# haidog-yaqub/EzAudio

Measured on AMD Instinct MI355X. Metric: denoising steps/sec (EzAudio-XL, 10 s latent, CFG on), higher is better.
Workload: dtype bf16

## Files before the change

ezaudio_amd/csrc/attn.hip:

```cpp
#include "common.h"

namespace {

typedef __attribute__((ext_vector_type(4))) short s16x4;

__device__ __forceinline__ float pair_max(float x) {
    const auto r = __builtin_amdgcn_permlane32_swap(__float_as_uint(x), __float_as_uint(x), false, false);
    return fmaxf(__uint_as_float(r[0]), __uint_as_float(r[1]));
}
__device__ __forceinline__ float pair_sum(float x) {
    const auto r = __builtin_amdgcn_permlane32_swap(__float_as_uint(x), __float_as_uint(x), false, false);
    return __uint_as_float(r[0]) + __uint_as_float(r[1]);
}

template <int DH>
struct HeadGeom;
template <>
struct HeadGeom<64> { static constexpr int DQK = 64, DV = 64; };
template <>
struct HeadGeom<72> { static constexpr int DQK = 80, DV = 96; };

template <int DH, int NKH, bool ZQ = false, int QT = 64>
__global__ __launch_bounds__(128 * NKH) void k_attn(AttnArgs a) {
    static_assert(QT == 64 || (QT == 32 && NKH == 4), "32-query tiles: the 8-wave fused-projection form only");
    constexpr int NQS = QT / 32;
    constexpr int NT = 128 * NKH;
    constexpr int TK = 32 * NKH;
    constexpr int DQK = HeadGeom<DH>::DQK;
    constexpr int DV = HeadGeom<DH>::DV;
    constexpr int NKS = DQK / 16;
    constexpr int NDT = DV / 32;
    constexpr int KSTR = DQK * 2 + 16;
    constexpr int VSTR = 192;
    static_assert(DV * 2 <= VSTR, "V row");
    constexpr int KBYTES = TK * KSTR, VBYTES = TK * VSTR;
    constexpr int BUF = KBYTES + VBYTES;
    constexpr int KCH = TK * DQK * 2 / 16;
    constexpr int VCPR = DV / 8;
    constexpr int VCH = TK * VCPR;
    constexpr int KPT = (KCH + NT - 1) / NT, VPT = (VCH + NT - 1) / NT;
    static_assert(KPT <= 3 && VPT <= 3, "staging registers");
    constexpr int DN = DV >= 96 ? 96 : 64;
    constexpr int DW = DQK;
    constexpr int DS = DQK;
    constexpr int NRS = QT == 64 ? 3 : 4;
    constexpr int PSTAGE = (QT + DN) * 128, PRING = 2 * NRS * PSTAGE;
    constexpr int PRED = 4 * 64 * DS * 4, PQS = QT * DQK * 2;
    constexpr int SMEM = NKH == 4 ? (2 * BUF > PRED + PQS ? (2 * BUF > PRING ? 2 * BUF : PRING) : (PRED + PQS > PRING ? PRED + PQS : PRING)) : 2 * BUF;
    constexpr int ZX = ZQ ? QT * 8 + 2 * DQK * 4 : 0;
    __shared__ __attribute__((aligned(16))) char smem[SMEM + ZX];

    int Lq_ = a.Lq;
    asm("" : "+s"(Lq_) : "s"(a.q), "s"(a.k), "s"(a.v), "s"(a.kmask), "s"(a.out), "s"(a.ldo), "s"(a.B), "s"(a.H), "s"(a.Lk), "s"(a.Lqp), "s"(a.Lkp), "s"(a.xu), "s"(a.ldu),
        "s"(a.xw), "s"(a.ldw), "s"(a.xw_rows), "s"(a.xK), "s"(a.xcd_map), "s"(a.nq), "s"(a.ppx), "s"(a.mnq), "s"(a.mH), "s"(a.q_raw), "s"(a.ts), "s"(a.xk2), "s"(a.zstat_in),
        "s"(a.zs_stride), "s"(a.zparts));
    const int tid = threadIdx.x;
    const int lane = tid & 63;
    const int wave = tid >> 6;
    const int qs = QT == 64 ? (wave & 1) : 0, kh = QT == 64 ? (wave >> 1) : (wave & 3);
    const bool active = QT == 64 || __builtin_amdgcn_readfirstlane(wave) < 4;
    const int r32 = lane & 31, hi = lane >> 5;
    int qt, h, b;
    if (a.xcd_map) {
        const int xcd = blockIdx.x & 7, sl = blockIdx.x >> 3;
        const int sq = ez_div(sl, a.mnq);
        const int pair = xcd * a.ppx + sq;
        qt = sl - sq * a.nq;
        if (pair >= a.B * a.H) return;
        b = ez_div(pair, a.mH); h = pair - b * a.H;
    } else {
        qt = blockIdx.x; h = blockIdx.y; b = blockIdx.z;
    }
    const int q0 = qt * QT + qs * 32;
    const long bh = (long)b * a.H + h;
    unsigned long long* ts = (a.ts && tid < 64) ? a.ts + 8 * (long)blockIdx.x : nullptr;
    if (ts && lane == 0) { ts[0] = __builtin_readcyclecounter(); ts[6] = ez_stamp_start(); }

    const bf16_t* Q = a.q + (bh * a.Lqp + q0 + r32) * DQK + 8 * hi;
    const char* Kg = reinterpret_cast<const char*>(a.k + bh * a.Lkp * DQK);
    const bf16_t* Vg = a.v + bh * DV * (long)a.Lkp;
    const uint8_t* km = a.kmask ? a.kmask + (long)b * a.Lk : nullptr;

    bf16x8 qf[NKS];
    if (NKH == 4 && a.xu) {
        if constexpr (NKH == 4) {
            constexpr int FN = DN / 32;
            constexpr int NPART = QT == 64 ? 4 : 8;
            const int rowb = b * a.Lq;
            float2* zrow_l = reinterpret_cast<float2*>(smem + SMEM);
            float* zgc_l = reinterpret_cast<float*>(smem + SMEM + QT * 8);
            ZStatRegs zst;
            float4 zgc_reg = make_float4(0.f, 0.f, 0.f, 0.f);
            const int wave_u = __builtin_amdgcn_readfirstlane(wave);
            const char* gA = reinterpret_cast<const char*>(a.xu);
            const char* gW = reinterpret_cast<const char*>(a.xw);
            const int nt = a.xK / 64;
            auto z_request = [&]() {
                if constexpr (ZQ) {
                    if (tid < 4 * QT) {
                        int qr = qt * QT + (tid >> 2);
                        qr = qr < a.Lq ? qr : a.Lq - 1;
                        z_row_stats_load(a.zstat_in + (rowb + qr), a.zs_stride, a.zparts, tid & 3, zst);
                    }
                    if (tid < 2 * (DH / 4)) {
                        const int which = tid >= DH / 4, t4 = tid - which * (DH / 4);
                        zgc_reg = *reinterpret_cast<const float4*>((which ? a.zC : a.zG) + h * DH + 4 * t4);
                    }
                }
            };
            f32x16 acc[FN];
#pragma unroll
            for (int j = 0; j < FN; ++j)
#pragma unroll
                for (int r = 0; r < 16; ++r) acc[j][r] = 0.f;
            if constexpr (QT == 32) {
                constexpr int NCH = (32 + DW) * 8, NW1 = (NCH - NT) / 64;
                static_assert(NCH > NT && NCH <= 2 * NT && (NCH - NT) % 64 == 0, "two passes, whole waves");
                uint32_t off0, off1;
                {
                    const int row = tid >> 3, c = tid & 7;
                    if (row < 32) {
                        int grow = rowb + qt * 32 + row;
                        grow = grow < rowb + a.Lq - 1 ? grow : rowb + a.Lq - 1;
                        off0 = (uint32_t)(grow * a.ldu + ((c ^ ((row >> 1) & 7)) << 3)) * 2u;
                    } else {
                        const int r2 = row - 32;
                        int gr = h * DH + r2;
                        gr = gr < a.xw_rows - 1 ? gr : a.xw_rows - 1;
                        off0 = (uint32_t)(gr * a.ldw + ((c ^ ((r2 >> 1) & 7)) << 3)) * 2u;
                    }
                    const int r2 = (tid >> 3) + 32;
                    int gr = h * DH + r2;
                    gr = gr < a.xw_rows - 1 ? gr : a.xw_rows - 1;
                    off1 = (uint32_t)(gr * a.ldw + ((c ^ ((r2 >> 1) & 7)) << 3)) * 2u;
                }
                const char* g0 = wave_u < 4 ? gA : gW;
                const bool two = wave_u < NW1;
                auto stage2 = [&](int sidx) {
                    char* dst = smem + (sidx % NRS) * 2 * PSTAGE + wave_u * 1024;
#pragma unroll
                    for (int sub = 0; sub < 2; ++sub) {
                        const long ko = (long)(2 * sidx + sub) * 128;
                        __builtin_amdgcn_global_load_lds((const __attribute__((address_space(1))) void*)(g0 + ko + off0),
                                                         (__attribute__((address_space(3))) void*)(dst + sub * PSTAGE), 16, 0, 0);
                        if (two)
                            __builtin_amdgcn_global_load_lds((const __attribute__((address_space(1))) void*)(gW + ko + off1),
                                                             (__attribute__((address_space(3))) void*)(dst + sub * PSTAGE + NT * 16), 16, 0, 0);
                    }
                };
                const int ns = nt >> 1;
                stage2(0);
                z_request();
                if (ns > 1) stage2(1);
                if (ns > 2) stage2(2);
                const int sub = wave_u >> 2, kq = wave_u & 3;
                const uint32_t fo = r32 * 128 + (((2 * kq + hi) ^ ((r32 >> 1) & 7)) << 4);
                for (int sidx = 0; sidx < ns; ++sidx) {
                    const int younger = ns - 1 - sidx < NRS - 2 ? ns - 1 - sidx : NRS - 2;
                    if (two) {
                        if (younger >= 2) asm volatile("s_waitcnt vmcnt(8)" ::: "memory");
                        else if (younger == 1) asm volatile("s_waitcnt vmcnt(4)" ::: "memory");
                        else asm volatile("s_waitcnt vmcnt(0)" ::: "memory");
                    } else {
                        if (younger >= 2) asm volatile("s_waitcnt vmcnt(4)" ::: "memory");
                        else if (younger == 1) asm volatile("s_waitcnt vmcnt(2)" ::: "memory");
                        else asm volatile("s_waitcnt vmcnt(0)" ::: "memory");
                    }
                    __builtin_amdgcn_s_barrier();
                    if (sidx + NRS - 1 < ns) stage2(sidx + NRS - 1);
                    const char* cT = smem + (sidx % NRS) * 2 * PSTAGE + sub * PSTAGE;
                    const bf16x8 af = *reinterpret_cast<const bf16x8*>(cT + fo);
#pragma unroll
                    for (int j = 0; j < FN; ++j) {
                        const bf16x8 bfr = *reinterpret_cast<const bf16x8*>(cT + 32 * 128 + fo + j * 4096);
                        acc[j] = __builtin_amdgcn_mfma_f32_32x32x16_bf16(bfr, af, acc[j], 0, 0, 0);
                    }
#pragma unroll
                    for (int j = 0; j < FN; ++j) asm volatile("" : "+a"(acc[j]));
                }
            } else {
            const int mh = wave & 1, kq = wave >> 1;
            uint32_t aoff[1], boff[(DW * 8 + NT - 1) / NT];
            stage_offsets<64, NT>(aoff, a.ldu, rowb + qt * 64, rowb + a.Lq - 1, tid);
            stage_offsets<DW, NT>(boff, a.ldw, h * DH, a.xw_rows - 1, tid);
            auto stage = [&](int t) {
                char* dst = smem + (t % 3) * PSTAGE + wave_u * 1024;
                stage_tile<64, NT>(gA + (long)t * 128, aoff, dst, tid);
                stage_tile<DW, NT>(gW + (long)t * 128, boff, dst + 64 * 128, tid);
            };
            const bool two = (DW * 8 > NT) && (wave_u * 64 + NT < DW * 8);
            stage(0);
            if (nt > 1) stage(1);
            z_request();
            const uint32_t fo = r32 * 128 + (((2 * kq + hi) ^ ((r32 >> 1) & 7)) << 4);
            if (a.xk2 && (nt & 1) == 0) {
                const int ns = nt >> 1;
                auto stage2 = [&](int sidx) {
                    char* dst = smem + (sidx % 3) * 2 * PSTAGE + wave_u * 1024;
#pragma unroll
                    for (int sub = 0; sub < 2; ++sub) {
                        stage_tile<64, NT>(gA + (long)(2 * sidx + sub) * 128, aoff, dst + sub * PSTAGE, tid);
                        stage_tile<DW, NT>(gW + (long)(2 * sidx + sub) * 128, boff, dst + sub * PSTAGE + 64 * 128, tid);
                    }
                };
                if (ns > 1) stage2(1);
                for (int sidx = 0; sidx < ns; ++sidx) {
                    if (sidx + 1 < ns) {
                        if (two) asm volatile("s_waitcnt vmcnt(6)" ::: "memory"); else asm volatile("s_waitcnt vmcnt(4)" ::: "memory");
                    } else {
                        asm volatile("s_waitcnt vmcnt(0)" ::: "memory");
                    }
                    __builtin_amdgcn_s_barrier();
                    if (sidx + 2 < ns) stage2(sidx + 2);
#pragma unroll
                    for (int sub = 0; sub < 2; ++sub) {
                        const char* cT = smem + (sidx % 3) * 2 * PSTAGE + sub * PSTAGE;
                        const bf16x8 af = *reinterpret_cast<const bf16x8*>(cT + fo + mh * 4096);
#pragma unroll
                        for (int j = 0; j < FN; ++j) {
                            const bf16x8 bfr = *reinterpret_cast<const bf16x8*>(cT + 64 * 128 + fo + j * 4096);
                            acc[j] = __builtin_amdgcn_mfma_f32_32x32x16_bf16(bfr, af, acc[j], 0, 0, 0);
                        }
                    }
#pragma unroll
                    for (int j = 0; j < FN; ++j) asm volatile("" : "+a"(acc[j]));
                }
            } else
            for (int t = 0; t < nt; ++t) {
                if (t + 1 < nt) {
                    if (two) asm volatile("s_waitcnt vmcnt(3)" ::: "memory"); else asm volatile("s_waitcnt vmcnt(2)" ::: "memory");
                } else {
                    asm volatile("s_waitcnt vmcnt(0)" ::: "memory");
                }
                __builtin_amdgcn_s_barrier();
                if (t + 2 < nt) stage(t + 2);
                const char* cT = smem + (t % 3) * PSTAGE;
                const bf16x8 af = *reinterpret_cast<const bf16x8*>(cT + fo + mh * 4096);
#pragma unroll
                for (int j = 0; j < FN; ++j) {
                    const bf16x8 bfr = *reinterpret_cast<const bf16x8*>(cT + 64 * 128 + fo + j * 4096);
                    acc[j] = __builtin_amdgcn_mfma_f32_32x32x16_bf16(bfr, af, acc[j], 0, 0, 0);
                }
#pragma unroll
                for (int j = 0; j < FN; ++j) asm volatile("" : "+a"(acc[j]));
            }
            }
#pragma unroll
            for (int j = 0; j < FN; ++j) asm volatile("s_nop 7\n\ts_nop 7\n\ts_nop 3" : "+a"(acc[j]));
            if constexpr (ZQ) {
                if (tid < 4 * QT) {
                    const float2 mr = z_row_stats_finish(zst, a.zparts, tid & 3, a.zD, a.zeps);
                    if ((tid & 3) == 0) zrow_l[tid >> 2] = mr;
                }
                if (tid < 2 * (DH / 4)) {
                    const int which = tid >= DH / 4, t4 = tid - which * (DH / 4);
                    *reinterpret_cast<float4*>(zgc_l + which * DQK + 4 * t4) = zgc_reg;
                }
            }
            __syncthreads();
            float* red = reinterpret_cast<float*>(smem);
            {
                const int pw = QT == 64 ? (wave >> 1) : wave, prow = QT == 64 ? 32 * (wave & 1) + r32 : r32;
#pragma unroll
                for (int j = 0; j < FN; ++j)
#pragma unroll
                    for (int g = 0; g < 4; ++g) {
                        const int col = 32 * j + 8 * g + 4 * hi;
                        if (col < DS)
                            *reinterpret_cast<float4*>(red + ((pw * QT + prow) * DS + col)) =
                                make_float4(acc[j][4 * g], acc[j][4 * g + 1], acc[j][4 * g + 2], acc[j][4 * g + 3]);
                    }
            }
            __syncthreads();
            if (QT == 64 || tid < 8 * QT) {
                constexpr int CP = DH / 8;
                bf16_t* qs_l = reinterpret_cast<bf16_t*>(smem + PRED);
                const int row = tid >> 3, part = tid & 7;
                float v[CP];
                float s1 = 0.f;
                const float2 zmr = ZQ ? zrow_l[row] : make_float2(0.f, 1.f);
                const float zmu = zmr.x, zr = zmr.y;
#pragma unroll
                for (int e = 0; e < CP; ++e) {
                    const int col = part * CP + e;
                    if constexpr (QT == 64) {
                        v[e] = red[(0 * 64 + row) * DS + col] + red[(1 * 64 + row) * DS + col] + red[(2 * 64 + row) * DS + col] +
                               red[(3 * 64 + row) * DS + col];
                    } else {
                        float t = red[row * DS + col];
#pragma unroll
                        for (int w = 1; w < NPART; ++w) t += red[(w * QT + row) * DS + col];
                        v[e] = t;
                    }
                    if constexpr (ZQ) v[e] = fmaf(zr, v[e], fmaf(-zr * zmu, zgc_l[col], zgc_l[DQK + col]));
                    s1 += v[e];
                }
                s1 = oct_sum(s1);
                const float mean = s1 * (1.f / DH);
                float s2 = 0.f;
#pragma unroll
                for (int e = 0; e < CP; ++e) { const float d = v[e] - mean; s2 += d * d; }
                s2 = oct_sum(s2);
                const float rstd = rsqrtf(s2 * (1.f / DH) + 1e-5f);
#pragma unroll
                for (int e = 0; e < CP; ++e) {
                    const int col = part * CP + e;
                    qs_l[row * DQK + col] = f2bf((v[e] - mean) * rstd * a.qn_w[col] + a.qn_b[col]);
                }
                if (DQK > DH && part == 0)
                    for (int col = DH; col < DQK; ++col) qs_l[row * DQK + col] = 0;
            }
            __syncthreads();
            {
                const bf16_t* qs_l = reinterpret_cast<const bf16_t*>(smem + PRED);
#pragma unroll
                for (int ks = 0; ks < NKS; ++ks) qf[ks] = *reinterpret_cast<const bf16x8*>(qs_l + (32 * qs + r32) * DQK + 16 * ks + 8 * hi);
            }
            __syncthreads();
        }
    } else if (a.q_raw) {
        int qr = q0 + r32;
        if (qr >= a.Lq) qr = a.Lq - 1;
        const float* src = a.q_raw + ((long)b * a.Lq + qr) * a.ld_qraw + h * DH + 8 * hi;
        float v[NKS][8];
        float s = 0.f;
#pragma unroll
        for (int ks = 0; ks < NKS; ++ks) {
            const bool ok = 16 * ks + 8 * hi < DH;
            const float4 lo = ok ? *reinterpret_cast<const float4*>(src + 16 * ks) : make_float4(0.f, 0.f, 0.f, 0.f);
            const float4 hh = ok ? *reinterpret_cast<const float4*>(src + 16 * ks + 4) : make_float4(0.f, 0.f, 0.f, 0.f);
            v[ks][0] = lo.x; v[ks][1] = lo.y; v[ks][2] = lo.z; v[ks][3] = lo.w;
            v[ks][4] = hh.x; v[ks][5] = hh.y; v[ks][6] = hh.z; v[ks][7] = hh.w;
#pragma unroll
            for (int e = 0; e < 8; ++e) s += v[ks][e];
        }
        s += __shfl_xor(s, 32, 64);
        const float mean = s * (1.f / DH);
        float q2 = 0.f;
#pragma unroll
        for (int ks = 0; ks < NKS; ++ks)
            if (16 * ks + 8 * hi < DH) {
#pragma unroll
                for (int e = 0; e < 8; ++e) { const float d = v[ks][e] - mean; q2 += d * d; }
            }
        q2 += __shfl_xor(q2, 32, 64);
        const float rstd = rsqrtf(q2 * (1.f / DH) + 1e-5f);
#pragma unroll
        for (int ks = 0; ks < NKS; ++ks) {
            const int d0 = 16 * ks + 8 * hi;
            const bool ok = d0 < DH;
            const int dw = ok ? d0 : 0;
            union { bf16x8 v; uint32_t u[4]; } pk;
#pragma unroll
            for (int e = 0; e < 4; ++e) {
                const float y0 = ok ? (v[ks][2 * e] - mean) * rstd * a.qn_w[dw + 2 * e] + a.qn_b[dw + 2 * e] : 0.f;
                const float y1 = ok ? (v[ks][2 * e + 1] - mean) * rstd * a.qn_w[dw + 2 * e + 1] + a.qn_b[dw + 2 * e + 1] : 0.f;
                pk.u[e] = pack_bf2(y0, y1);
            }
            qf[ks] = pk.v;
        }
    } else {
#pragma unroll
        for (int ks = 0; ks < NKS; ++ks) qf[ks] = *reinterpret_cast<const bf16x8*>(Q + 16 * ks);
    }

    uint4 k0 = {}, k1 = {}, k2 = {}, v0 = {}, v1 = {}, v2 = {};
    uint32_t koff[3], voff[3];
#pragma unroll
    for (int i = 0; i < 3; ++i) {
        int ck = tid + NT * i, cv = tid + NT * i;
        ck = ck < KCH ? ck : KCH - 1;
        cv = cv < VCH ? cv : VCH - 1;
        koff[i] = (uint32_t)ck * 16u;
        voff[i] = (uint32_t)cv * 16u;
    }
    const __amdgpu_buffer_rsrc_t krs = __builtin_amdgcn_make_buffer_rsrc(const_cast<char*>(Kg), 0, a.Lkp * DQK * 2, 0x00020000);
    const __amdgpu_buffer_rsrc_t vrs = __builtin_amdgcn_make_buffer_rsrc(const_cast<bf16_t*>(Vg), 0, DV * a.Lkp * 2, 0x00020000);
    auto kchunk = [&](int i, int key0) -> uint4 {
        return __builtin_bit_cast(uint4, __builtin_amdgcn_raw_buffer_load_b128(krs, (int)koff[i], key0 * DQK * 2, 0));
    };
    auto vchunk = [&](int i, int key0) -> uint4 {
        return __builtin_bit_cast(uint4, __builtin_amdgcn_raw_buffer_load_b128(vrs, (int)voff[i], key0 * DV * 2, 0));
    };
    auto kstore = [&](int i, char* kb, const uint4& val) {
        const int c = tid + NT * i;
        if (c < KCH) *reinterpret_cast<uint4*>(kb + (c / (DQK / 8)) * KSTR + (c % (DQK / 8)) * 16) = val;
    };
    auto vstore = [&](int i, char* vb, const uint4& val) {
        const int c = tid + NT * i;
        if (c < VCH) *reinterpret_cast<uint4*>(vb + (c / VCPR) * VSTR + (c % VCPR) * 16) = val;
    };
#define LOAD_TILE(t)                                   \
    do {                                               \
        const int key0_ = (t) * TK;                    \
        k0 = kchunk(0, key0_);                         \
        k1 = kchunk(1, key0_);                         \
        if constexpr (KPT > 2) k2 = kchunk(2, key0_);  \
        v0 = vchunk(0, key0_);                         \
        v1 = vchunk(1, key0_);                         \
        if constexpr (VPT > 2) v2 = vchunk(2, key0_);  \
    } while (0)
#define WRITE_TILE(buf)                                \
    do {                                               \
        char* kb_ = smem + (buf) * BUF;                \
        char* vb_ = kb_ + KBYTES;                      \
        kstore(0, kb_, k0);                            \
        kstore(1, kb_, k1);                            \
        if constexpr (KPT > 2) kstore(2, kb_, k2);     \
        vstore(0, vb_, v0);                            \
        vstore(1, vb_, v1);                            \
        if constexpr (VPT > 2) vstore(2, vb_, v2);     \
    } while (0)

    f32x16 o[NDT];
#pragma unroll
    for (int t = 0; t < NDT; ++t)
#pragma unroll
        for (int r = 0; r < 16; ++r) o[t][r] = 0.f;
    float m = -1e30f, lsum = 0.f;
    constexpr float RESCALE_THR = 4.0f;
    const float c = 1.4426950408889634f * rsqrtf((float)DH);

    if (NKH == 4 && __builtin_amdgcn_readfirstlane(threadIdx.x) >= 256) __builtin_amdgcn_s_setprio(1);
    const int ntiles = (a.Lk + TK - 1) / TK;
    LOAD_TILE(0);
    WRITE_TILE(0);
    __syncthreads();
    if (ts && lane == 0) ts[1] = __builtin_readcyclecounter();
    for (int t = 0; t < ntiles; ++t) {
        if (t + 1 < ntiles) LOAD_TILE(t + 1);
        const char* kb = smem + (t & 1) * BUF;
        const char* vb = kb + KBYTES;
        const char* vtr = vb + (32 * kh + 4 * hi + ((lane & 15) >> 2)) * VSTR + ((lane & 16) + 4 * (lane & 3)) * 2;
        const int key0 = t * TK + kh * 32;
        if (active && key0 < a.Lk) {
            const int kidx = key0 + r32;
            bool kv = kidx < a.Lk;
            if (km) kv = kv && (km[kidx < a.Lk ? kidx : 0] != 0);
            const uint32_t ball = (uint32_t)__ballot(kv);
            const uint32_t tmask = ball >> (4 * hi);
            const bool full = ball == 0xffffffffu;
            f32x16 s;
            {
                const bf16x8 kf0 = *reinterpret_cast<const bf16x8*>(kb + (kh * 32 + r32) * KSTR + hi * 16);
                asm("s_nop 1\n\tv_mfma_f32_32x32x16_bf16 %0, %1, %2, 0" : "=&v"(s) : "v"(kf0), "v"(qf[0]));
            }
#pragma unroll
            for (int ks = 1; ks < NKS; ++ks) {
                const bf16x8 kf = *reinterpret_cast<const bf16x8*>(kb + (kh * 32 + r32) * KSTR + (2 * ks + hi) * 16);
                if (ks + 1 < NKS) asm("s_nop 1\n\tv_mfma_f32_32x32x16_bf16 %0, %1, %2, %0" : "+v"(s) : "v"(kf), "v"(qf[ks]));
                else asm("s_nop 1\n\tv_mfma_f32_32x32x16_bf16 %0, %1, %2, %0\n\ts_nop 7\n\ts_nop 7\n\ts_nop 3" : "+v"(s) : "v"(kf), "v"(qf[ks]));
            }
            float tmax = -1e30f;
            if (full) {
#pragma unroll
                for (int r = 0; r < 16; ++r) tmax = fmaxf(tmax, s[r]);
                tmax *= c;
            } else {
#pragma unroll
                for (int r = 0; r < 16; ++r) {
                    const bool v = (tmask >> ((r & 3) + 8 * (r >> 2))) & 1u;
                    s[r] = v ? s[r] * c : -1e30f;
                    tmax = fmaxf(tmax, s[r]);
                }
            }
            tmax = pair_max(tmax);
            if (!__all(tmax <= m + RESCALE_THR)) {
                const float mnew = fmaxf(m, tmax);
                const float alpha = __builtin_amdgcn_exp2f(m - mnew);
                m = mnew;
                lsum *= alpha;
#pragma unroll
                for (int tt = 0; tt < NDT; ++tt)
#pragma unroll
                    for (int r = 0; r < 16; ++r) o[tt][r] *= alpha;
            }
            float psum = 0.f;
            float p[16];
            if (full) {
                const f32x2 c2 = {c, c}, nm2 = {-m, -m};
                f32x2 ps2 = {0.f, 0.f};
#pragma unroll
                for (int r = 0; r < 16; r += 2) {
                    f32x2 x = {s[r], s[r + 1]};
                    x = __builtin_elementwise_fma(x, c2, nm2);
                    p[r] = __builtin_amdgcn_exp2f(x[0]);
                    p[r + 1] = __builtin_amdgcn_exp2f(x[1]);
                    const f32x2 pp = {p[r], p[r + 1]};
                    ps2 += pp;
                }
                psum = ps2[0] + ps2[1];
            } else {
#pragma unroll
                for (int r = 0; r < 16; ++r) {
                    const bool v = (tmask >> ((r & 3) + 8 * (r >> 2))) & 1u;
                    p[r] = v ? __builtin_amdgcn_exp2f(s[r] - m) : 0.f;
                    psum += p[r];
                }
            }
            psum = pair_sum(psum);
            lsum += psum;
#pragma unroll
            for (int step = 0; step < 2; ++step) {
                union { bf16x8 v; uint32_t u[4]; } pf;
#pragma unroll
                for (int e = 0; e < 4; ++e) pf.u[e] = pack_bf2(p[8 * step + 2 * e], p[8 * step + 2 * e + 1]);
#pragma unroll
                for (int tt = 0; tt < NDT; ++tt) {
                    const char* vp = vtr + (16 * step) * VSTR + 64 * tt;
                    union { bf16x8 v; s16x4 h2[2]; } vf;
                    vf.h2[0] = __builtin_amdgcn_ds_read_tr16_b64_v4i16((__attribute__((address_space(3))) s16x4*)(vp));
                    vf.h2[1] = __builtin_amdgcn_ds_read_tr16_b64_v4i16((__attribute__((address_space(3))) s16x4*)(vp + 8 * VSTR));
                    asm("s_nop 1\n\tv_mfma_f32_32x32x16_bf16 %0, %1, %2, %0" : "+v"(o[tt]) : "v"(vf.v), "v"(pf.v));
                }
            }
        }
        if (t + 1 < ntiles) WRITE_TILE((t + 1) & 1);
        __syncthreads();
    }

    if (ts && lane == 0) ts[2] = __builtin_readcyclecounter();
#pragma unroll
    for (int tt = 0; tt < NDT; ++tt) asm volatile("s_nop 7\n\ts_nop 7\n\ts_nop 3" : "+v"(o[tt]));
    constexpr int NG = DH / 8;
    constexpr int NW = 2 * NKH;
    float4* xo = reinterpret_cast<float4*>(smem);
    float* xml = reinterpret_cast<float*>(smem + NKH * NQS * NG * 64 * 16);
    static_assert(SMEM >= NKH * NQS * NG * 64 * 16 + NKH * NQS * 2 * 32 * 4, "exchange area must fit the staging buffers");
    if (active) {
#pragma unroll
        for (int G = 0; G < NG; ++G)
            xo[((kh * NQS + qs) * NG + G) * 64 + lane] = make_float4(o[G / 4][4 * (G % 4)], o[G / 4][4 * (G % 4) + 1], o[G / 4][4 * (G % 4) + 2], o[G / 4][4 * (G % 4) + 3]);
        if (hi == 0) {
            xml[((kh * NQS + qs) * 2 + 0) * 32 + r32] = m;
            xml[((kh * NQS + qs) * 2 + 1) * 32 + r32] = lsum;
        }
    }
    __syncthreads();
    if (ts && lane == 0) ts[4] = __builtin_readcyclecounter();
    float wgt[NKH];
    {
        float mk[NKH], mm = -1e30f;
#pragma unroll
        for (int k = 0; k < NKH; ++k) { mk[k] = xml[((k * NQS + qs) * 2 + 0) * 32 + r32]; mm = fmaxf(mm, mk[k]); }
        float l = 0.f;
#pragma unroll
        for (int k = 0; k < NKH; ++k) { wgt[k] = __builtin_amdgcn_exp2f(mk[k] - mm); l = fmaf(xml[((k * NQS + qs) * 2 + 1) * 32 + r32], wgt[k], l); }
        const float inv = 1.f / l;
#pragma unroll
        for (int k = 0; k < NKH; ++k) wgt[k] *= inv;
    }
    const int qrow = q0 + r32;
    bf16_t* orow = a.out + ((long)b * a.Lq + (qrow < a.Lq ? qrow : a.Lq - 1)) * a.ldo + h * DH + 4 * hi;
#pragma unroll
    for (int i = 0; i < (NQS * NG + NW - 1) / NW; ++i) {
        const int G = (wave + i * NW) / NQS;
        if (G < NG) {
            float4 acc = make_float4(0.f, 0.f, 0.f, 0.f);
#pragma unroll
            for (int k = 0; k < NKH; ++k) {
                const float4 v = xo[((k * NQS + qs) * NG + G) * 64 + lane];
                acc.x = fmaf(v.x, wgt[k], acc.x); acc.y = fmaf(v.y, wgt[k], acc.y); acc.z = fmaf(v.z, wgt[k], acc.z); acc.w = fmaf(v.w, wgt[k], acc.w);
            }
            if (qrow < a.Lq) {
                uint2 v;
                v.x = pack_bf2(acc.x, acc.y);
                v.y = pack_bf2(acc.z, acc.w);
                if (a.wt) st8_wt(orow + 8 * G, v); else *reinterpret_cast<uint2*>(orow + 8 * G) = v;
            }
        }
    }
    if (ts && lane == 0) { asm volatile("s_waitcnt vmcnt(0)" ::: "memory"); ts[3] = __builtin_readcyclecounter(); ts[7] = __builtin_amdgcn_s_memrealtime(); }
}

#undef LOAD_TILE
#undef WRITE_TILE

}

int launch_attention(const AttnArgs& a0, hipStream_t st) {
    AttnArgs a = a0;
    if (a.b0 > 0) {
        const int DQK = a.dh == 64 ? 64 : 80, DV = a.dh == 64 ? 64 : 96;
        const long b0 = a.b0;
        if (a.q) a.q += b0 * a.H * a.Lqp * DQK;
        if (a.k) a.k += b0 * a.H * a.Lkp * DQK;
        if (a.v) a.v += b0 * a.H * DV * (long)a.Lkp;
        if (a.kmask) a.kmask += b0 * a.Lk;
        if (a.out) a.out += b0 * a.Lq * a.ldo;
        if (a.q_raw) a.q_raw += b0 * a.Lq * a.ld_qraw;
        if (a.xu) a.xu += b0 * a.Lq * a.ldu;
        if (a.zstat_in) a.zstat_in += b0 * a.Lq;
        a.b0 = 0;
    }
    const long nwg64 = (long)((a.Lq + 63) / 64) * a.H * a.B;
    int nkh = a.nkh;
    if (nkh != 2 && nkh != 4) nkh = nwg64 <= 512 ? 4 : 2;
    if (a.Lkp % 128) nkh = 2;
    if (a.xu && nkh != 4) return 1;
    if (a.dh != 64 && a.dh != 72) return 1;
    const bool zq = a.xu && a.zstat_in;
    if (zq && !(a.zG && a.zC && a.zparts > 0 && a.zparts <= Z_MAXP && a.zs_stride > 0 && a.zw > 0)) return 1;
    const bool q32 = zq && nkh == 4 && (a.xK / 64) % 2 == 0 && a.xcd_map && (a.qtile == 32 || (a.qtile == 0 && nwg64 <= 128));
    const int QT = q32 ? 32 : 64;
    a.nq = (a.Lq + QT - 1) / QT;
    a.ppx = (a.B * a.H + 7) / 8;
    a.mnq = ez_magic(a.nq); a.mH = ez_magic(a.H);
    dim3 grid(a.nq, a.H, a.B);
    if (a.xcd_map) grid = dim3(8 * a.ppx * a.nq, 1, 1);
    if (a.ts && (long)grid.x * grid.y * grid.z > a.ts_cap) a.ts = nullptr;
    if (q32) {
        if (a.dh == 64) hipLaunchKernelGGL((k_attn<64, 4, true, 32>), grid, dim3(512), 0, st, a);
        else hipLaunchKernelGGL((k_attn<72, 4, true, 32>), grid, dim3(512), 0, st, a);
        return 0;
    }
    if (a.dh == 64) {
        if (nkh == 4 && zq) hipLaunchKernelGGL((k_attn<64, 4, true>), grid, dim3(512), 0, st, a);
        else if (nkh == 4) hipLaunchKernelGGL((k_attn<64, 4>), grid, dim3(512), 0, st, a);
        else hipLaunchKernelGGL((k_attn<64, 2>), grid, dim3(256), 0, st, a);
    } else {
        if (nkh == 4 && zq) hipLaunchKernelGGL((k_attn<72, 4, true>), grid, dim3(512), 0, st, a);
        else if (nkh == 4) hipLaunchKernelGGL((k_attn<72, 4>), grid, dim3(512), 0, st, a);
        else hipLaunchKernelGGL((k_attn<72, 2>), grid, dim3(256), 0, st, a);
    }
    return 0;
}
```

Before: 263.6.

## Restructure fused Q-projection staging into per-wave k-chunks with barrier-free pipelining

For the 32-query fused projection path, each wave now owns whole 64-wide k-chunks in its own LDS slot, with two waves double-buffered. This replaces the shared 3/4-stage ring that needed a block barrier every step. All fragment reads are issued before the next chunk's async global-to-LDS load, and the z-statistics loads are folded into the vmcnt accounting. The cross-wave partial-sum reduction moves to a swizzled float4 layout with vectorized reads and packed bf16 stores, and one syncthreads is dropped. Explicit s_nop padding after the MFMAs adds fixed stall cycles, and the more complex vmcnt bookkeeping risks subtle ordering bugs.

```diff
diff --git a/ezaudio_amd/csrc/attn.hip b/ezaudio_amd/csrc/attn.hip
--- a/ezaudio_amd/csrc/attn.hip
+++ b/ezaudio_amd/csrc/attn.hip
@@ -43,10 +43,17 @@
     constexpr int DN = DV >= 96 ? 96 : 64;
     constexpr int DW = DQK;
     constexpr int DS = DQK;
-    constexpr int NRS = QT == 64 ? 3 : 4;
-    constexpr int PSTAGE = (QT + DN) * 128, PRING = 2 * NRS * PSTAGE;
-    constexpr int PRED = 4 * 64 * DS * 4, PQS = QT * DQK * 2;
-    constexpr int SMEM = NKH == 4 ? (2 * BUF > PRED + PQS ? (2 * BUF > PRING ? 2 * BUF : PRING) : (PRED + PQS > PRING ? PRED + PQS : PRING)) : 2 * BUF;
+    constexpr int PSTAGE = (64 + DN) * 128, PRING = 2 * 3 * PSTAGE;
+    constexpr int NPC = (32 + DW) / 8;
+    constexpr int CHUNK = NPC * 1024, SLOT = (32 + DN) * 128, NX = 2;
+    constexpr int PSLOTS = 8 * SLOT + NX * CHUNK + (DN - DW) * 128;
+    constexpr int RP = 24;
+    constexpr int PPART = QT == 64 ? 64 * RP * 16 : SLOT;
+    constexpr int PRED = QT == 64 ? 4 * PPART : 8 * SLOT, PQS = QT * DQK * 2;
+    static_assert(QT == 64 || 32 * RP * 16 <= SLOT, "a wave's partial tile must fit its slot");
+    static_assert(DS / 4 <= RP && RP % 8 == 0, "partial rows");
+    constexpr int PPROJ = QT == 64 ? (PRED + PQS > PRING ? PRED + PQS : PRING) : (PSLOTS > PRED + PQS ? PSLOTS : PRED + PQS);
+    constexpr int SMEM = NKH == 4 ? (2 * BUF > PPROJ ? 2 * BUF : PPROJ) : 2 * BUF;
     constexpr int ZX = ZQ ? QT * 8 + 2 * DQK * 4 : 0;
     __shared__ __attribute__((aligned(16))) char smem[SMEM + ZX];
 
@@ -108,75 +115,88 @@
                     }
                 }
             };
+            auto z_request_all = [&]() {
+                if constexpr (ZQ) {
+                    int qr = qt * QT + ((tid >> 2) & (QT - 1));
+                    qr = qr < a.Lq ? qr : a.Lq - 1;
+                    z_row_stats_load(a.zstat_in + (rowb + qr), a.zs_stride, a.zparts, tid & 3, zst);
+                    const int tc = tid < 2 * (DH / 4) ? tid : 2 * (DH / 4) - 1;
+                    const int which = tc >= DH / 4, t4 = tc - which * (DH / 4);
+                    zgc_reg = *reinterpret_cast<const float4*>((which ? a.zC : a.zG) + h * DH + 4 * t4);
+                }
+            };
             f32x16 acc[FN];
 #pragma unroll
             for (int j = 0; j < FN; ++j)
 #pragma unroll
                 for (int r = 0; r < 16; ++r) acc[j][r] = 0.f;
             if constexpr (QT == 32) {
-                constexpr int NCH = (32 + DW) * 8, NW1 = (NCH - NT) / 64;
-                static_assert(NCH > NT && NCH <= 2 * NT && (NCH - NT) % 64 == 0, "two passes, whole waves");
-                uint32_t off0, off1;
-                {
-                    const int row = tid >> 3, c = tid & 7;
-                    if (row < 32) {
+                constexpr int NZ = ZQ ? Z_PT + 1 : 0;
+                static_assert(NZ + NPC < 64, "vmcnt is a 6-bit counter");
+                uint32_t poff[NPC];
+#pragma unroll
+                for (int p = 0; p < NPC; ++p) {
+                    const int row = 8 * p + (lane >> 3), c = lane & 7;
+                    if (p < 4) {
                         int grow = rowb + qt * 32 + row;
                         grow = grow < rowb + a.Lq - 1 ? grow : rowb + a.Lq - 1;
-                        off0 = (uint32_t)(grow * a.ldu + ((c ^ ((row >> 1) & 7)) << 3)) * 2u;
+                        poff[p] = (uint32_t)(grow * a.ldu + ((c ^ ((row >> 1) & 7)) << 3)) * 2u;
                     } else {
                         const int r2 = row - 32;
                         int gr = h * DH + r2;
                         gr = gr < a.xw_rows - 1 ? gr : a.xw_rows - 1;
-                        off0 = (uint32_t)(gr * a.ldw + ((c ^ ((r2 >> 1) & 7)) << 3)) * 2u;
-                    }
-                    const int r2 = (tid >> 3) + 32;
-                    int gr = h * DH + r2;
-                    gr = gr < a.xw_rows - 1 ? gr : a.xw_rows - 1;
-                    off1 = (uint32_t)(gr * a.ldw + ((c ^ ((r2 >> 1) & 7)) << 3)) * 2u;
-                }
-                const char* g0 = wave_u < 4 ? gA : gW;
-                const bool two = wave_u < NW1;
-                auto stage2 = [&](int sidx) {
-                    char* dst = smem + (sidx % NRS) * 2 * PSTAGE + wave_u * 1024;
-#pragma unroll
-                    for (int sub = 0; sub < 2; ++sub) {
-                        const long ko = (long)(2 * sidx + sub) * 128;
-                        __builtin_amdgcn_global_load_lds((const __attribute__((address_space(1))) void*)(g0 + ko + off0),
-                                                         (__attribute__((address_space(3))) void*)(dst + sub * PSTAGE), 16, 0, 0);
-                        if (two)
-                            __builtin_amdgcn_global_load_lds((const __attribute__((address_space(1))) void*)(gW + ko + off1),
-                                                             (__attribute__((address_space(3))) void*)(dst + sub * PSTAGE + NT * 16), 16, 0, 0);
-                    }
+                        poff[p] = (uint32_t)(gr * a.ldw + ((c ^ ((r2 >> 1) & 7)) << 3)) * 2u;
+                    }
+                }
+                auto issue = [&](int c, char* dst) {
+                    const long ko = (long)c * 128;
+#pragma unroll
+                    for (int p = 0; p < NPC; ++p)
+                        __builtin_amdgcn_global_load_lds((const __attribute__((address_space(1))) void*)((p < 4 ? gA : gW) + ko + poff[p]),
+                                                         (__attribute__((address_space(3))) void*)(dst + p * 1024), 16, 0, 0);
                 };
-                const int ns = nt >> 1;
-                stage2(0);
-                z_request();
-                if (ns > 1) stage2(1);
-                if (ns > 2) stage2(2);
-                const int sub = wave_u >> 2, kq = wave_u & 3;
-                const uint32_t fo = r32 * 128 + (((2 * kq + hi) ^ ((r32 >> 1) & 7)) << 4);
-                for (int sidx = 0; sidx < ns; ++sidx) {
-                    const int younger = ns - 1 - sidx < NRS - 2 ? ns - 1 - sidx : NRS - 2;
-                    if (two) {
-                        if (younger >= 2) asm volatile("s_waitcnt vmcnt(8)" ::: "memory");
-                        else if (younger == 1) asm volatile("s_waitcnt vmcnt(4)" ::: "memory");
+                const int nmine = wave_u < nt ? (nt - wave_u + 7) >> 3 : 0;
+                const bool two = wave_u < NX;
+                char* const slot0 = smem + wave_u * SLOT;
+                char* const slot1 = smem + 8 * SLOT + (two ? wave_u : 0) * CHUNK;
+                if (nmine > 0) issue(wave_u, slot0);
+                __builtin_amdgcn_sched_barrier(0);
+                z_request_all();
+                __builtin_amdgcn_sched_barrier(0);
+                if (two && nmine > 1) issue(wave_u + 8, slot1);
+                __builtin_amdgcn_sched_barrier(0);
+                uint32_t fo[4];
+#pragma unroll
+                for (int ks = 0; ks < 4; ++ks) fo[ks] = r32 * 128 + (((2 * ks + hi) ^ ((r32 >> 1) & 7)) << 4);
+                for (int i = 0; i < nmine; ++i) {
+                    const bool nxt = two && i + 1 < nmine;
+                    if (i == 0) {
+                        if (nxt) asm volatile("s_waitcnt vmcnt(%0)" ::"n"(NZ + NPC) : "memory");
+                        else asm volatile("s_waitcnt vmcnt(%0)" ::"n"(NZ) : "memory");
+                    } else {
+                        if (nxt) asm volatile("s_waitcnt vmcnt(%0)" ::"n"(NPC) : "memory");
                         else asm volatile("s_waitcnt vmcnt(0)" ::: "memory");
-                    } else {
-                        if (younger >= 2) asm volatile("s_waitcnt vmcnt(4)" ::: "memory");
-                        else if (younger == 1) asm volatile("s_waitcnt vmcnt(2)" ::: "memory");
-                        else asm volatile("s_waitcnt vmcnt(0)" ::: "memory");
-                    }
-                    __builtin_amdgcn_s_barrier();
-                    if (sidx + NRS - 1 < ns) stage2(sidx + NRS - 1);
-                    const char* cT = smem + (sidx % NRS) * 2 * PSTAGE + sub * PSTAGE;
-                    const bf16x8 af = *reinterpret_cast<const bf16x8*>(cT + fo);
-#pragma unroll
-                    for (int j = 0; j < FN; ++j) {
-                        const bf16x8 bfr = *reinterpret_cast<const bf16x8*>(cT + 32 * 128 + fo + j * 4096);
-                        acc[j] = __builtin_amdgcn_mfma_f32_32x32x16_bf16(bfr, af, acc[j], 0, 0, 0);
-                    }
-#pragma unroll
-                    for (int j = 0; j < FN; ++j) asm volatile("" : "+a"(acc[j]));
+                    }
+                    char* cur = (two && (i & 1)) ? slot1 : slot0;
+                    bf16x8 af[4], bfr[4][FN];
+#pragma unroll
+                    for (int ks = 0; ks < 4; ++ks) {
+                        af[ks] = *reinterpret_cast<const bf16x8*>(cur + fo[ks]);
+#pragma unroll
+                        for (int j = 0; j < FN; ++j) bfr[ks][j] = *reinterpret_cast<const bf16x8*>(cur + 32 * 128 + fo[ks] + j * 4096);
+                    }
+                    __builtin_amdgcn_sched_barrier(0);
+                    asm volatile("s_waitcnt lgkmcnt(0)" ::: "memory");
+                    __builtin_amdgcn_sched_barrier(0);
+                    const int step = two ? 2 : 1;
+                    if (i + step < nmine) issue(wave_u + 8 * (i + step), cur);
+                    __builtin_amdgcn_sched_barrier(0);
+#pragma unroll
+                    for (int ks = 0; ks < 4; ++ks)
+#pragma unroll
+                        for (int j = 0; j < FN; ++j) acc[j] = __builtin_amdgcn_mfma_f32_32x32x16_bf16(bfr[ks][j], af[ks], acc[j], 0, 0, 0);
+                    if constexpr (FN == 3) asm volatile("s_nop 7\n\ts_nop 7\n\ts_nop 3" : "+a"(acc[0]), "+a"(acc[1]), "+a"(acc[2]));
+                    else asm volatile("s_nop 7\n\ts_nop 7\n\ts_nop 3" : "+a"(acc[0]), "+a"(acc[1]));
                 }
             } else {
             const int mh = wave & 1, kq = wave >> 1;
@@ -222,8 +242,8 @@
                             acc[j] = __builtin_amdgcn_mfma_f32_32x32x16_bf16(bfr, af, acc[j], 0, 0, 0);
                         }
                     }
-#pragma unroll
-                    for (int j = 0; j < FN; ++j) asm volatile("" : "+a"(acc[j]));
+                    if constexpr (FN == 3) asm volatile("s_nop 7\n\ts_nop 7\n\ts_nop 3" : "+a"(acc[0]), "+a"(acc[1]), "+a"(acc[2]));
+                    else asm volatile("s_nop 7\n\ts_nop 7\n\ts_nop 3" : "+a"(acc[0]), "+a"(acc[1]));
                 }
             } else
             for (int t = 0; t < nt; ++t) {
@@ -241,8 +261,8 @@
                     const bf16x8 bfr = *reinterpret_cast<const bf16x8*>(cT + 64 * 128 + fo + j * 4096);
                     acc[j] = __builtin_amdgcn_mfma_f32_32x32x16_bf16(bfr, af, acc[j], 0, 0, 0);
                 }
-#pragma unroll
-                for (int j = 0; j < FN; ++j) asm volatile("" : "+a"(acc[j]));
+                    if constexpr (FN == 3) asm volatile("s_nop 7\n\ts_nop 7\n\ts_nop 3" : "+a"(acc[0]), "+a"(acc[1]), "+a"(acc[2]));
+                    else asm volatile("s_nop 7\n\ts_nop 7\n\ts_nop 3" : "+a"(acc[0]), "+a"(acc[1]));
             }
             }
 #pragma unroll
@@ -257,41 +277,49 @@
                     *reinterpret_cast<float4*>(zgc_l + which * DQK + 4 * t4) = zgc_reg;
                 }
             }
-            __syncthreads();
-            float* red = reinterpret_cast<float*>(smem);
+            if constexpr (QT == 64) __syncthreads();
+            float4* red4 = reinterpret_cast<float4*>(smem);
             {
                 const int pw = QT == 64 ? (wave >> 1) : wave, prow = QT == 64 ? 32 * (wave & 1) + r32 : r32;
 #pragma unroll
                 for (int j = 0; j < FN; ++j)
 #pragma unroll
                     for (int g = 0; g < 4; ++g) {
-                        const int col = 32 * j + 8 * g + 4 * hi;
-                        if (col < DS)
-                            *reinterpret_cast<float4*>(red + ((pw * QT + prow) * DS + col)) =
+                        const int cu = 8 * j + 2 * g + hi;
+                        if (4 * (8 * j + 2 * g) < DS)
+                            red4[pw * (PPART / 16) + prow * RP + (cu ^ (prow & 7))] =
                                 make_float4(acc[j][4 * g], acc[j][4 * g + 1], acc[j][4 * g + 2], acc[j][4 * g + 3]);
                     }
             }
             __syncthreads();
             if (QT == 64 || tid < 8 * QT) {
+                static_assert(DH == 64 || DH == 72, "column ownership of phase 1b");
                 constexpr int CP = DH / 8;
                 bf16_t* qs_l = reinterpret_cast<bf16_t*>(smem + PRED);
                 const int row = tid >> 3, part = tid & 7;
+                const float4* p0 = red4 + row * RP;
+                const int u0 = part ^ (row & 7), u2 = (16 + (part >> 2)) ^ (row & 7);
+                float4 t0 = p0[u0], t1 = p0[8 + u0], t2 = make_float4(0.f, 0.f, 0.f, 0.f);
+                if constexpr (DH > 64) t2 = p0[u2];
+#pragma unroll
+                for (int w = 1; w < NPART; ++w) {
+                    const float4* pwp = p0 + w * (PPART / 16);
+                    const float4 x0 = pwp[u0], x1 = pwp[8 + u0];
+                    t0.x += x0.x; t0.y += x0.y; t0.z += x0.z; t0.w += x0.w;
+                    t1.x += x1.x; t1.y += x1.y; t1.z += x1.z; t1.w += x1.w;
+                    if constexpr (DH > 64) { const float4 x2 = pwp[u2]; t2.x += x2.x; t2.y += x2.y; t2.z += x2.z; t2.w += x2.w; }
+                }
                 float v[CP];
+                v[0] = t0.x; v[1] = t0.y; v[2] = t0.z; v[3] = t0.w;
+                v[4] = t1.x; v[5] = t1.y; v[6] = t1.z; v[7] = t1.w;
+                if constexpr (DH > 64) { const int e = part & 3; v[CP - 1] = e == 0 ? t2.x : e == 1 ? t2.y : e == 2 ? t2.z : t2.w; }
+                auto col_of = [&](int e) { return e < 4 ? 4 * part + e : e < 8 ? 32 + 4 * part + (e - 4) : 64 + part; };
                 float s1 = 0.f;
                 const float2 zmr = ZQ ? zrow_l[row] : make_float2(0.f, 1.f);
                 const float zmu = zmr.x, zr = zmr.y;
 #pragma unroll
                 for (int e = 0; e < CP; ++e) {
-                    const int col = part * CP + e;
-                    if constexpr (QT == 64) {
-                        v[e] = red[(0 * 64 + row) * DS + col] + red[(1 * 64 + row) * DS + col] + red[(2 * 64 + row) * DS + col] +
-                               red[(3 * 64 + row) * DS + col];
-                    } else {
-                        float t = red[row * DS + col];
-#pragma unroll
-                        for (int w = 1; w < NPART; ++w) t += red[(w * QT + row) * DS + col];
-                        v[e] = t;
-                    }
+                    const int col = col_of(e);
                     if constexpr (ZQ) v[e] = fmaf(zr, v[e], fmaf(-zr * zmu, zgc_l[col], zgc_l[DQK + col]));
                     s1 += v[e];
                 }
@@ -302,11 +330,15 @@
                 for (int e = 0; e < CP; ++e) { const float d = v[e] - mean; s2 += d * d; }
                 s2 = oct_sum(s2);
                 const float rstd = rsqrtf(s2 * (1.f / DH) + 1e-5f);
+                float y[CP];
 #pragma unroll
                 for (int e = 0; e < CP; ++e) {
-                    const int col = part * CP + e;
-                    qs_l[row * DQK + col] = f2bf((v[e] - mean) * rstd * a.qn_w[col] + a.qn_b[col]);
-                }
+                    const int col = col_of(e);
+                    y[e] = (v[e] - mean) * rstd * a.qn_w[col] + a.qn_b[col];
+                }
+                *reinterpret_cast<uint2*>(qs_l + row * DQK + 4 * part) = make_uint2(pack_bf2(y[0], y[1]), pack_bf2(y[2], y[3]));
+                *reinterpret_cast<uint2*>(qs_l + row * DQK + 32 + 4 * part) = make_uint2(pack_bf2(y[4], y[5]), pack_bf2(y[6], y[7]));
+                if constexpr (DH > 64) qs_l[row * DQK + 64 + part] = f2bf(y[CP - 1]);
                 if (DQK > DH && part == 0)
                     for (int col = DH; col < DQK; ++col) qs_l[row * DQK + col] = 0;
             }
```

After: 264.9, median of 6. No clear change (+0.5%).
